# Hongje/OTVM

Hardware: AMD Instinct MI355X
Metric: frames_per_sec (higher is better)
Workload: dtype f16x3 (fp32 operands split into fp16 hi+lo, fp32 accumulate); 1 GPU; synthetic 1920x1080 clip, T=140 frames (untimed lead-in 0 + warmup 5 + timed: the last 135), memory every 5, max 5 slots, trimap propagation + alpha + memorize per frame, one sequence per GPU; weights=synthetic (otvm_amd.synth_weights seed 0), parallelism=sequence-per-gpu x1, batch=1

## Files before the change

### include/otvm_hip.h

```cpp
#ifndef OTVM_HIP_H
#define OTVM_HIP_H

#include <stdint.h>

#ifdef __cplusplus
extern "C" {
#endif

#define OTVM_ACT_NONE 0
#define OTVM_ACT_RELU 1
#define OTVM_ACT_LEAKY 2

#define OTVM_PREC_F32 0
#define OTVM_PREC_F16X3 1
#define OTVM_PREC_F16 2

const char* otvm_last_error(void);
#define OTVM_ABI_VERSION 21
int otvm_abi_version(void);

int otvm_pack_conv_weight(const float* w_oihw, int O, int I, int kh, int kw, int ws, const float* scale,
                          float* w_packed, int O_pad, int I_pad, int K_pad, void* stream);

int64_t otvm_patch_weight_bytes_f16x3(int O, int I_pad);
// ... 58 lines not shown
int otvm_conv2d_candidates(const otvm_conv_params* p, int* out, int max_n);
int otvm_conv2d_accepts_input_norm(const otvm_conv_params* p);
int otvm_conv2d_input_norm_kind(const otvm_conv_params* p);

typedef struct otvm_conv_up_params {
    const float* src; int Hi, Wi, Cu, src_ld;
    int64_t src_bs;
    const float* scale; const float* shift;
    int act;
    int norm_bs;
    int tile_rows;
} otvm_conv_up_params;
int otvm_conv2d_up(const otvm_conv_params* p, const otvm_conv_up_params* u, void* stream);
int otvm_conv2d_accepts_upsampled_input(const otvm_conv_params* p, const otvm_conv_up_params* u);

int otvm_split_conv_weight_f16x3(const float* w_packed, int O, int O_pad, int K_pad, int taps, int I_pad,
                                 void* w_hi, void* w_lo, float* w_scale, void* stream);

int64_t otvm_wave_weight_bytes_f16x3(int O_pad, int K_pad);
int otvm_pack_wave_weight_f16x3(const void* w_hi, const void* w_lo, int O_pad, int K_pad, void* w_wfrag, void* stream);

typedef struct {
    const float* x; int H, W, Cin, x_ld;
    float* y; int y_ld;
    const void* w1f; const void* w2f; const void* w3f;
    const float* s1; const float* s2; const float* s3;
    const float* b1; const float* b2; const float* b3;
    int batch; int64_t x_bs, y_bs;
    int tile;
} otvm_stm_bottleneck_params;
// ... 4 lines not shown
                  float* shift, void* stream);
int otvm_gn_apply(const float* x, int64_t P, int C, int ld, const double* stats, const float* gamma,
                  const float* beta, const float* residual, int res_ld, const float* res_scale, const float* res_shift,
                  int res_act, int act, float* out, int out_ld, void* stream);

int otvm_gn_stats_b(const float* x, int64_t P, int C, int ld, double* stats, int batch, int64_t x_bs, int stats_bs, void* stream);
int otvm_gn_table_b(const double* stats, int64_t P, int C, const float* gamma, const float* beta, float* scale, float* shift,
                    int batch, int stats_bs, int norm_bs, void* stream);
typedef struct {
    const float* x; int64_t P; int C, ld; const double* stats; const float* gamma; const float* beta;
    const float* residual; int res_ld; const float* res_scale; const float* res_shift; int res_act, act;
    float* out; int out_ld;
    int batch; int64_t x_bs, res_bs, out_bs; int stats_bs, norm_bs;
} otvm_gn_apply_params;
int otvm_gn_apply_b(const otvm_gn_apply_params* p, void* stream);

typedef struct otvm_gram_params {
    const float* x; int64_t P; int C, ld;
    const float* in_scale; const float* in_shift; int in_act;
    float* gpart; float* spart; int passes;
    int batch; int64_t x_bs; int norm_bs;
    unsigned* diag;
} otvm_gram_params;
int otvm_gram_block(int C);
int64_t otvm_gram_entries(int C);
int otvm_gram_chunks(int64_t P, int C, int* pch_out);
int otvm_gram_f16(const otvm_gram_params* p, void* stream);
typedef struct otvm_gn_predict_params {
    const float* gpart; const float* spart; int64_t P; int C, Cout;
    const float* Mp; const double* v; void* ws; unsigned* counter;
// ... 270 lines not shown
```

### otvm_amd/csrc/conv_stem_f16x3.hip

```cpp
#include "common.h"
#include "f16x3_ops.h"
#include <type_traits>
#include <stdlib.h>

namespace {

struct StemArgs {
    const float* in; const _Float16* wf; const float* wscale; const float* bias; float* out; double* gn_stats;
    int H, W, Cin, in_ld, Ho, Wo, Cout, out_ld, act, groups;
    int tiles_x, tiles_y; OtvmTileWalk walk;
    int64_t in_bs, out_bs; int gn_bs;
    OtvmGnTail tail;
};

constexpr int TH = 8, TW = 32, NW = 4, NT = NW * 64;
constexpr int TM = TH / NW, TN = 2;
constexpr int PH = 2 * TH + 5, PW = 2 * TW + 5, NPIX = PH * PW;
constexpr int KSTEPS = 25;

__global__ __launch_bounds__(NT) __attribute__((amdgpu_waves_per_eu(2, 2))) void conv_stem_f16x3_kernel(const StemArgs pa) {
    StemArgs p = pa;
    {
        const int zb = blockIdx.y;
        p.in += zb * p.in_bs;
        p.out += zb * p.out_bs;
        if (p.gn_stats) p.gn_stats += zb * p.gn_bs;
    }
    constexpr int PATCH_HALFS = 2 * NPIX * 8;
    constexpr int EPI_HALFS = NW * 32 * 36 * 2;
    constexpr int SM_HALFS = PATCH_HALFS > EPI_HALFS ? PATCH_HALFS : EPI_HALFS;
    __shared__ __attribute__((aligned(16))) _Float16 smem[SM_HALFS];
    _Float16* Ph = smem;
    _Float16* Pl = smem + NPIX * 8;

    const int tid = threadIdx.x, lane = tid & 63, wave = tid >> 6;
    int tile_n_, tile_x, tile_y;
    otvm_tile_decode(p.walk, blockIdx.x, gridDim.x, 1, p.tiles_x, p.tiles_y, tile_n_, tile_x, tile_y);
    const int ty0 = tile_y * TH, tx0 = tile_x * TW;
    const int iy00 = 2 * ty0 - 3, ix00 = 2 * tx0 - 3;

    f32x16 acc[TM][TN];
// ... 151 lines not shown
                        const int64_t m = (int64_t)y * p.Wo + x;
                        if (FULL || (vec_ok && n4 + 3 < p.Cout)) {
                            v.x = otvm_act(v.x, p.act); v.y = otvm_act(v.y, p.act);
                            v.z = otvm_act(v.z, p.act); v.w = otvm_act(v.w, p.act);
                            *reinterpret_cast<f32x4*>(p.out + m * p.out_ld + n4) = v;
                        } else {
#pragma unroll
                            for (int j = 0; j < 4; ++j)
                                if (n4 + j < p.Cout) p.out[m * p.out_ld + n4 + j] = otvm_act(v[j], p.act);
                        }
                    }
                }
            }
        }
    };
    if (interior) {
        if (p.act == OTVM_ACT_RELU) epilogue_full(std::integral_constant<int, OTVM_ACT_RELU>{});
        else if (p.act == OTVM_ACT_LEAKY) epilogue_full(std::integral_constant<int, OTVM_ACT_LEAKY>{});
        else epilogue_full(std::integral_constant<int, OTVM_ACT_NONE>{});
    } else {
        epilogue(std::false_type{});
    }
    if (p.gn_stats) {
        __shared__ double gred[2 * 64];
        const int cg = p.Cout >> 5;
        const int seg = cg < 32 ? cg : 32;
        for (int i = tid; i < 2 * 64; i += NT) gred[i] = 0.0;
        __syncthreads();
#pragma unroll
        for (int b = 0; b < TN; ++b) {
            const int n = b * 32 + col;
            float s = 0.f, ss = 0.f, cnt = 0.f;
            const float pil = n < p.Cout && p.bias ? p.bias[n / cg * cg] : 0.f;
            if (n < p.Cout) {
                const float sc_ = p.wscale[n];
                const float bias = p.bias ? p.bias[n] : 0.f, bd = bias - pil;
// ... 25 lines not shown
                double S, SS;
                otvm_gn_unshift(s, ss, (int)cnt, pil, S, SS);
                atomicAdd(&gred[2 * gl], S);
                atomicAdd(&gred[2 * gl + 1], SS);
            }
        }
        __syncthreads();
        const int ng = (64 + cg - 1) / cg;
        for (int i = tid; i < 2 * ng; i += NT) {
            const int g = i >> 1;
            if (g < 32 && gred[i] != 0.0) atomicAdd(&p.gn_stats[2 * g + (i & 1)], gred[i]);
        }
        __syncthreads();
        otvm_gn_table_tail(p.gn_stats, (int64_t)p.Ho * p.Wo, p.Cout, p.tail, blockIdx.y, gridDim.x, reinterpret_cast<float*>(gred));
    }
}

__global__ __launch_bounds__(256) void pack_stem_weight_kernel(const float* __restrict__ w, int O, int K_pad, int I_pad, int groups,
                                                               _Float16* __restrict__ wf, float* __restrict__ wscale) {
    const int n = blockIdx.x;
    __shared__ float red[256];
    const bool real = n < O;
    const float* row = w + (int64_t)n * K_pad;
    float mx = 0.f;
    if (real)
        for (int k = threadIdx.x; k < 49 * I_pad; k += 256) mx = fmaxf(mx, fabsf(row[k]));
    red[threadIdx.x] = mx;
    __syncthreads();
    for (int s = 128; s > 0; s >>= 1) {
        if (threadIdx.x < s) red[threadIdx.x] = fmaxf(red[threadIdx.x], red[threadIdx.x + s]);
// ... 38 lines not shown
                   p->Cin <= 64 && !p->residual && !p->in_relu && !p->in_scale ? 1 : 0;
}

int otvm_conv2d_stem_f16x3(const otvm_conv_params* p, void* stream) {
    StemArgs a;
    a.in = p->in; a.wf = (const _Float16*)p->w_frag; a.wscale = p->w_scale; a.bias = p->bias; a.out = p->out;
    a.gn_stats = p->gn_stats;
    a.tail = otvm_gn_tail_of(p);
    a.H = p->H; a.W = p->W; a.Cin = p->Cin; a.in_ld = p->in_ld; a.Ho = p->Ho; a.Wo = p->Wo; a.Cout = p->Cout;
    a.out_ld = p->out_ld; a.act = p->act; a.groups = (p->Cin + 7) / 8;
    a.tiles_x = otvm_ceil_div(p->Wo, TW);
    a.tiles_y = otvm_ceil_div(p->Ho, TH);
    a.walk = otvm_tile_walk_of(2);
    const int batch = p->batch > 1 ? p->batch : 1;
    a.in_bs = batch > 1 ? p->in_bs : 0; a.out_bs = batch > 1 ? p->out_bs : 0; a.gn_bs = batch > 1 ? p->gn_bs : 0;
    hipLaunchKernelGGL(conv_stem_f16x3_kernel, dim3(a.tiles_x * a.tiles_y, batch), dim3(NT), 0, (hipStream_t)stream, a);
    OTVM_CHECK_LAUNCH("otvm_conv2d(stem f16x3)");
    return 0;
}
```

### otvm_amd/csrc/groupnorm.hip

```cpp
#include "common.h"
#include "f16x3_ops.h"
#include <stdlib.h>

namespace {

constexpr int G = 32;

__global__ void gn_stats_kernel(const float* __restrict__ x, int64_t P, int C, int ld, double* __restrict__ stats,
                                int64_t x_bs, int stats_bs) {
    x += blockIdx.y * x_bs;
    stats += blockIdx.y * stats_bs;
    __shared__ double red[G * 2];
    const int Q = C >> 2;
    const int rows = blockDim.x / Q;
    const int q = threadIdx.x % Q, r = threadIdx.x / Q;
    if (threadIdx.x < G * 2) red[threadIdx.x] = 0.0;
    __syncthreads();
    f32x4 s = {0.f, 0.f, 0.f, 0.f}, ss = {0.f, 0.f, 0.f, 0.f}, p0 = {0.f, 0.f, 0.f, 0.f};
    int n = 0;
    const int64_t pix0 = (int64_t)blockIdx.x * rows + r, step = (int64_t)gridDim.x * rows;
    if (r < rows && pix0 < P) {
        p0 = *reinterpret_cast<const f32x4*>(x + pix0 * ld + q * 4);
        n = (int)((P - 1 - pix0) / step) + 1;
        int64_t pix = pix0 + step;
// ... 81 lines not shown
        rb = *reinterpret_cast<const f32x4*>(res_shift + c);
    }
    for (; pix < P; pix += dpix) {
        f32x4 v = *reinterpret_cast<const f32x4*>(x + pix * ld + c);
        v = v * a + b;
        if (residual) {
            f32x4 r = *reinterpret_cast<const f32x4*>(residual + pix * res_ld + c);
            if (res_scale) {
                r = r * ra + rb;
                r.x = otvm_act(r.x, res_act); r.y = otvm_act(r.y, res_act); r.z = otvm_act(r.z, res_act); r.w = otvm_act(r.w, res_act);
            }
            v += r;
        }
        v.x = otvm_act(v.x, act); v.y = otvm_act(v.y, act); v.z = otvm_act(v.z, act); v.w = otvm_act(v.w, act);
        *reinterpret_cast<f32x4*>(out + pix * out_ld + c) = v;
    }
}

__global__ void gn_table_kernel(const double* __restrict__ stats, int64_t P, int C, const float* __restrict__ gamma,
                                const float* __restrict__ beta, float* __restrict__ scale, float* __restrict__ shift,
                                int stats_bs, int norm_bs) {
    stats += blockIdx.x * stats_bs;
    scale += blockIdx.x * norm_bs;
    shift += blockIdx.x * norm_bs;
    __shared__ float mean_s[G], rstd_s[G];
    const int cg = C / G;
    if (threadIdx.x < G) {
        const double cnt = (double)P * cg;
        const double mean = stats[threadIdx.x * 2] / cnt;
        double var = stats[threadIdx.x * 2 + 1] / cnt - mean * mean;
// ... 61 lines not shown
    const int64_t total = q->P * Q;
    int64_t blocks = (total + 255) / 256;
    if (blocks > 4096) blocks = 4096;
    int gcd = 256, r = Q;
    while (r) { const int t = gcd % r; gcd = r; r = t; }
    const int m = Q / gcd;
    blocks = (blocks + m - 1) / m * m;
    const bool b = batch > 1;
    hipLaunchKernelGGL(gn_apply_kernel, dim3((int)blocks, batch), dim3(256), 0, (hipStream_t)stream, q->x, q->P, C, q->ld, q->stats,
                       q->gamma, q->beta, q->residual, q->res_ld, q->res_scale, q->res_shift, q->res_act, q->act, q->out, q->out_ld,
                       b ? q->x_bs : 0, b ? q->res_bs : 0, b ? q->out_bs : 0, b ? q->stats_bs : 0, b ? q->norm_bs : 0);
    OTVM_CHECK_LAUNCH("otvm_gn_apply");
    return 0;
}

extern "C" int otvm_gn_apply(const float* x, int64_t P, int C, int ld, const double* stats, const float* gamma,
                             const float* beta, const float* residual, int res_ld, const float* res_scale,
                             const float* res_shift, int res_act, int act, float* out, int out_ld, void* stream) {
    otvm_gn_apply_params q;
    q.x = x; q.P = P; q.C = C; q.ld = ld; q.stats = stats; q.gamma = gamma; q.beta = beta; q.residual = residual; q.res_ld = res_ld;
    q.res_scale = res_scale; q.res_shift = res_shift; q.res_act = res_act; q.act = act; q.out = out; q.out_ld = out_ld;
    q.batch = 1; q.x_bs = q.res_bs = q.out_bs = 0; q.stats_bs = q.norm_bs = 0;
    return otvm_gn_apply_b(&q, stream);
}
```

### otvm_amd/engine.py

```python
import ctypes as C
import os

import torch

from . import lib as L

NONE, RELU, LEAKY = 0, 1, 2
GUARD_CLEAR = 2 ** 31 - 1
F16_LIMIT = 65504.0
FUSE_GN_STATS = True
FUSE_GN_APPLY = os.environ.get("OTVM_FUSE_GN_APPLY", "1") != "0"
_GRAPHS_ENV = os.environ.get("OTVM_GRAPHS")
USE_GRAPHS = None if _GRAPHS_ENV in (None, "", "auto") else (_GRAPHS_ENV != "0")
GRAPH_AUTO_PIXELS = 1 << 22


def graphs_wanted(setting, padded_pixels):
    if setting is not None:
        return bool(setting)
    if int(os.environ.get("WORLD_SIZE", "1")) > 1:
        return True
    return padded_pixels < GRAPH_AUTO_PIXELS
PRE_ON_S2 = os.environ.get("OTVM_PRE_ON_S2", "1") != "0"
EVDEC_LATE = os.environ.get("OTVM_EVDEC_LATE", "1") != "0"
WAVE_TILE = os.environ.get("OTVM_WAVE_TILE", "0") != "0"
FUSE_GN_APPLY_IGEMM = os.environ.get("OTVM_FUSE_GN_APPLY_IGEMM", "1") != "0"
FUSE_GN_APPLY_IGEMM_KXK = os.environ.get("OTVM_FUSE_GN_APPLY_IGEMM_KXK", "0") != "0"
FUSE_GN_TABLE = os.environ.get("OTVM_FUSE_GN_TABLE", "1") != "0"
FUSE_STM_BLOCK = os.environ.get("OTVM_FUSE_STM_BLOCK", "1") != "0"
FUSE_STM_BLOCK128 = int(os.environ.get("OTVM_FUSE_STM_BLOCK128", "1"))
STM128_TILE = int(os.environ.get("OTVM_STM128_TILE", "0"))
FOLD_UPSAMPLE = int(os.environ.get("OTVM_FOLD_UPSAMPLE", "1"))
FUSE_PPM_HEAD = os.environ.get("OTVM_PPM_HEAD", "1") != "0"
FUSE_GN_PREDICT = os.environ.get("OTVM_GN_PREDICT", "1") != "0"
GN_PREDICT_MIN_PIXELS = int(os.environ.get("OTVM_GN_PREDICT_MIN_PIXELS", "16384"))
GN_PREDICT_PASSES = int(os.environ.get("OTVM_GN_PREDICT_PASSES", "1"))
GN_PREDICT_PLANES = tuple(int(v) for v in os.environ.get("OTVM_GN_PREDICT_PLANES", "64,128,256,512").split(",") if v)
GN_PREDICT_DS = os.environ.get("OTVM_GN_PREDICT_DS", "1") != "0"
GN_PREDICT_KAPPA_P3 = float(os.environ.get("OTVM_GN_PREDICT_KAPPA_P3", "4"))
GN_PREDICT_KAPPA_OFF = float(os.environ.get("OTVM_GN_PREDICT_KAPPA_OFF", "256"))
FUSE_REFINE_TAIL = os.environ.get("OTVM_FUSE_REFINE_TAIL", "0") != "0"
FUSE_HEAD = os.environ.get("OTVM_FUSE_HEAD", "1") != "0"
HEAD16 = os.environ.get("OTVM_HEAD16", "1") != "0"
PPM_ALGEBRA = os.environ.get("OTVM_PPM_ALGEBRA", "1") != "0"


AUTOTUNE = os.environ.get("OTVM_AUTOTUNE", "1") != "0"
# ... 948 lines not shown
        self.H, self.W, self.B = H, W, B
        self.fgr = bool(eng._fgr_on)
        if B > 1 and eng.precision != L.PREC_F16X3:
            raise NotImplementedError("otvm_amd: batched sequences (B > 1) run on the f16x3 path only")
        self.lw, self.uw, self.lh, self.uh = pad_amounts(H, W, 32)
        self.Hp, self.Wp = H + self.lh + self.uh, W + self.lw + self.uw
        self.P = self.Hp * self.Wp
        self._bufs = {}
        self._keep = []
        self.graphs, self._graph_warm = {}, {}
        self._n_conv = {}
        self._retired_graphs = []
        self._stm128 = []
        self._upfold = []
        self.upfold_routes = {}
        self._fused_stats = []
        self._convs = []
        self._predicted = []
        self.diag = None
        self.n_gn = 0
        self.steps = {}
        self._build()
        self.stats_bs = max(self.n_gn, 1) * 64
        self.stats = torch.zeros(self.B * self.stats_bs, dtype=torch.float64, device=self.dev)
        self._bind_stats()
        self.autotune()

    @staticmethod
    def _signature(p):
        return (p.H, p.W, p.Cin, p.in_ld, p.Cout, p.out_ld, p.kh, p.kw, p.stride, p.pad, p.dil, p.in_relu, p.act, int(bool(p.bias)),
# ... 44 lines not shown
                                 forced=(STM128_TILE or -1) if FUSE_STM_BLOCK128 >= 2 else None, default=None if timed else -1)
                if choice == 0:
                    S[i:i + 1] = U
                    i += len(U)
                else:
                    q.tile = max(choice, 0)
                    S[i] = fused
                    i += 1
        self._stm128 = []
        _save_choices_timed_since(n_logged)

    def autotune(self):
        if not (AUTOTUNE and self.e.precision == L.PREC_F16X3):
            self._resolve_stm128(timed=False)
            self._resolve_upfold(timed=False)
            return
        filled = []
        gen = torch.Generator(device=self.dev)
        gen.manual_seed(0x07F3)
        for b in self._bufs.values():
            t = b.t if isinstance(b, Act) else b
            if not t.is_floating_point():
                continue
            if t.dtype == torch.float32:
                t.normal_(generator=gen)
            else:
                continue
            filled.append(t)
        H16, W16 = self.Hp // 16, self.Wp // 16
        tk = Act(torch.empty(self.B * self.hw * 128, dtype=torch.float32, device=self.dev), H16, W16, 128, B=self.B, bs=self.hw * 128)
        tv = Act(torch.empty(self.B * self.hw * 512, dtype=torch.float32, device=self.dev), H16, W16, 512, B=self.B, bs=self.hw * 512)
        n0, k0 = len(self._convs), len(self._keep)
        self.conv([], self.r4m, "trimap.model.KV_M_r4.Key", tk, pad=1)
        self.conv([], self.r4m, "trimap.model.KV_M_r4.Value", tv, pad=1)
        self.tune_convs(self._convs)
        self._resolve_stm128(timed=FUSE_STM_BLOCK128 == 1)
        torch.cuda.synchronize(self.dev)
        del self._convs[n0:], self._keep[k0:]
        self._resolve_upfold(timed=FOLD_UPSAMPLE == 1)
        torch.cuda.synchronize(self.dev)
        for t in filled:
            t.zero_()
        self.stats.zero_()
        torch.cuda.synchronize(self.dev)

    def retire_graphs(self):
        self._retired_graphs.extend(self.graphs.values())
        self.graphs, self._graph_warm = {}, {}

    def clear_stats(self, stream):
        L.check(self.lib.otvm_clear(self.stats.data_ptr(), self.stats.numel() * 8, stream), "clear GroupNorm statistics")

    def buf(self, name, H, W, C):
        key = (name, H, W, C)
# ... 122 lines not shown
        for key, S in self.steps.items():
            for i, st in enumerate(S):
                if st[0] == "gn_stats":
                    _, a, idx, (nb, x_bs), label = st
                    S[i] = (self.lib.otvm_gn_stats_b, a + (base + idx * 512, nb, x_bs, sbs), label)
                elif st[0] == "gn_table":
                    _, a, idx, nbs, label = st
                    S[i] = (self.lib.otvm_gn_table_b, (base + idx * 512,) + a + (self.B, sbs, nbs), label)
                elif st[0] == "ppm_add":
                    _, a, b, label = st
                    S[i] = (self.lib.otvm_ppm_conv_add, a + (self._ppm_stats.gn_stats + 8 * b * sbs,), label)
                elif st[0] == "gn_apply":
                    _, q, idx, label = st
                    q.stats, q.stats_bs = base + idx * 512, sbs
                    S[i] = (self.lib.otvm_gn_apply_b, (C.byref(q),), label)

    def upsample(self, S, x, out, add=None, norm=None):
        S.append((self.lib.otvm_upsample_bilinear_b,
                  (x.ptr, x.H, x.W, x.C, x.ld, 0 if norm is None else norm[0], 0 if norm is None else norm[1],
                   0 if norm is None else norm[2], 0 if add is None else add.ptr, 0 if add is None else add.ld,
                   out.ptr, out.H, out.W, out.ld, x.B, x.bs, 0 if add is None else add.bs, out.bs,
                   0 if norm is None else norm[3]), "upsample"))

    def gn_then_upsample(self, S, x, gn_name, gn_act, producer_p, out):
        if FUSE_GN_APPLY and FUSE_GN_STATS and producer_p is not None:
            sc, sh, nbs = self.gn_table_step(S, x, gn_name, producer_p)
            self.upsample(S, x, out, norm=(sc, sh, gn_act, nbs))
            m = {"name": gn_name, "S": S, "step": S[-1], "src": x, "norm": (sc, sh, gn_act, nbs), "out": out, "readers": []}
            self._upfold.append(m)
            return m
# ... 31 lines not shown
                             lambda: _time_candidates(self.e, _EventClock(self.dev), routes.get, (0, 1) * 4, 3, warm=(0, 0, 1, 1)),
                             forced=1 if FOLD_UPSAMPLE >= 2 else None, default=None if timed else 0)
            if choice:
                at = lambda S, st: next(i for i, q in enumerate(S) if q is st)
                del m["S"][at(m["S"], m["step"])]
                for (S, step, p, x, wname), fs in zip(m["readers"], folded):
                    S[at(S, step)] = fs
                self.upfold_routes[m["name"]] = 1
                for b in range(max(1, m["out"].B)):
                    m["out"].torch(b).zero_()
        self._upfold = []
        _save_choices_timed_since(n_logged)

    def maxpool(self, S, x, out):
        S.append((self.lib.otvm_maxpool3x3s2_b, (x.ptr, x.H, x.W, x.C, x.ld, out.ptr, out.ld, x.B, x.bs, out.bs), "maxpool"))

    def gn_bottleneck(self, S, x, p, planes, stride, dil, has_ds, out):
        Ho, Wo = x.H // stride, x.W // stride
        t1 = self.buf("bt1", x.H, x.W, planes)
        cp = self.conv(S, x, p + ".conv1", t1)
        t2 = self.buf("bt2", Ho, Wo, planes)
        cp = self.gn_then_conv(S, t1, p + ".bn1", RELU, cp, p + ".conv2", t2, stride=stride, pad=dil, dil=dil)
        if self._predicted_tail(S, x, p, planes, stride, has_ds, out, t2, cp):
            return
        t3 = self.buf("bt3", Ho, Wo, planes * 4)
        if FUSE_GN_APPLY_IGEMM:
            cp3 = self.gn_then_conv(S, t2, p + ".bn2", RELU, cp, p + ".conv3", t3)
        else:
            self.gn(S, t2, p + ".bn2", RELU, conv_p=cp)
            cp3 = self.conv(S, t2, p + ".conv3", t3)
# ... 105 lines not shown
        self.conv(U, t2, p + ".conv3", out, residual=idt, act=RELU)
        if fuse128:
            q = L.StmBottleneckParams(x.ptr, x.H, x.W, x.C, x.ld, out.ptr, out.ld,
                                      c1.w_wfrag.data_ptr(), c2.w_wfrag.data_ptr(), c3.w_wfrag.data_ptr(),
                                      c1.w_scale.data_ptr(), c2.w_scale.data_ptr(), c3.w_scale.data_ptr(),
                                      c1.bias.data_ptr(), c2.bias.data_ptr(), c3.bias.data_ptr(), x.B, x.bs, out.bs, 0)
            self._keep.append(q)
            P = x.B * x.H * x.W
            flops = 2 * P * (512 * 128 + 9 * 128 * 128 + 128 * 512)
            abytes = 4 * (P * 512 * 2 + 512 * 128 * 2 + 9 * 128 * 128)
            fused = (self.lib.otvm_stm_bottleneck_f16x3, (C.byref(q),), "conv " + p + " (fused bottleneck)", flops, abytes,
                     (x, out.ch(0, 512) if out.C > 512 else out))
            S.append(("stm128", fused, U, q, p))
            self._stm128.append(S)

    def stm_trunk(self, S, stem_out, e, tag):
        H4, W4 = self.Hp // 4, self.Wp // 4
        x = self.buf(tag + "pool", H4, W4, 64)
        self.maxpool(S, stem_out, x)
        outs = {}
        for lname, n, planes, s0 in (("res2", 3, 64, 1), ("res3", 4, 128, 2), ("res4", 6, 256, 2)):
            for b in range(n):
                st = s0 if b == 0 else 1
                o = self.buf(tag + lname + ("a" if b % 2 == 0 else "b"), x.H // st, x.W // st, planes * 4)
                self.bn_bottleneck(S, x, e + "%s.%d" % (lname, b), planes, st, b == 0, o, tag)
                x = o
            outs[lname] = x
        return outs["res4"], outs["res3"], outs["res2"]

    def resblock(self, S, x, p, out, tag):
        r = self.buf(tag + "r", x.H, x.W, 256)
        self.conv(S, x, p + ".conv1", r, pad=1, in_relu=1)
        self.conv(S, r, p + ".conv2", out, pad=1, in_relu=1, residual=x)

# ... 9 lines not shown
        self.SQ = self.buf("SQ", Hp, Wp, 4)
        self.SMs = [self.buf("SM0", Hp, Wp, 24), self.buf("SM1", Hp, Wp, 24)]
        self.D80 = self.buf("D80", Hp, Wp, 80)
        self.PROBS_B = self.raws("probs", 3 * P)
        self.CLS_B = self.raws("cls", P, torch.uint8)
        self.ALPHA_P_B = self.raws("alpha_p", P)
        self.TRI_P_B = self.raws("tri_p", 3 * P)
        self.FGR_P_B = self.raws("fgr_p", 3 * P) if self.fgr else None
        self.enc_ws_B = self.raws("enc_ws", _rup(int(lib.otvm_trimap_encode_ws_bytes(Hp, Wp)), 256), torch.uint8)
        self.PROBS, self.CLS, self.ALPHA_P, self.TRI_P = self.PROBS_B[0], self.CLS_B[0], self.ALPHA_P_B[0], self.TRI_P_B[0]

        S = []
        sd = e.sd
        q = "trimap.model.Encoder_Q."
        stem = self.buf("q_stem", H2, W2, 64)
        self.conv(S, self.SQ, q + "conv1", stem, stride=2, pad=3, act=RELU)
        r4, r3, r2 = self.stm_trunk(S, stem, q, "q_")
        self.QK = self.buf("QK", H16, W16, 128)
        self.M4 = self.buf("M4", H16, W16, 1024)
        self.conv(S, r4, "trimap.model.KV_Q_r4.Key", self.QK, pad=1)
        self.conv(S, r4, "trimap.model.KV_Q_r4.Value", self.M4.ch(512, 512), pad=1)
        self.steps["segment_a"] = S
        self._ws = self.SPLITK_WS[0]
        S = []
        d = "trimap.model.Decoder."
        SK = []
        self._ws = self.SPLITK_WS[3]
        skips = {}
        for rf, feat, (h, w) in (("RF3", r3, (H8, W8)), ("RF2", r2, (H4, W4))):
            s0 = self.buf("d_s0", h, w, 256)
            self.conv(SK, feat, d + rf + ".convFS", s0, pad=1)
            s1 = self.buf("d_s1", h, w, 256)
# ... 15 lines not shown
        self.L4 = self.buf("L4", H4, W4, 4)
        self.conv(S, pm, d + "pred", self.L4, pad=1, in_relu=1)
        for b in range(self.B):
            S.append((lib.otvm_upsample4_softmax3, (self.L4.img(b).ptr, H4, W4, self.L4.ld, self.PROBS_B[b].data_ptr()), "up4softmax"))
        self.steps["segment_b"] = S

        S = []
        en = "NET.encoder."
        self.U3 = self.buf("U3", H2, W2, 320)
        self.U2 = self.buf("U2", H4, W4, 512)
        ppm_alg = FUSE_PPM_HEAD and self.e.W_ppm is not None
        self.PPMCAT = self.buf("PPMCAT", H8, W8, 2048 if ppm_alg else 3072)
        c1raw = self.buf("c1raw", H2, W2, 64)
        cp = self.conv(S, self.X11, en + "conv1", c1raw, stride=2, pad=3)
        c1 = self.U3.ch(256, 64)
        self.gn(S, c1raw, en + "bn1", RELU, out=c1, conv_p=cp)
        x = self.buf("e_pool", H4, W4, 64)
        self.maxpool(S, c1, x)
        cfg = {"layer1": (64, 3, 1, 1, 1), "layer2": (128, 4, 2, 1, 1), "layer3": (256, 6, 1, 1, 2),
               "layer4": (512, 3, 1, 2, 4)}
        for lname in ("layer1", "layer2", "layer3", "layer4"):
            planes, n, s0, d0, dn = cfg[lname]
            for b in range(n):
                st = s0 if b == 0 else 1
                last = b == n - 1
                if last and lname == "layer1":
                    o = self.U2.ch(256, 256)
                elif last and lname == "layer4":
                    o = self.PPMCAT.ch(0, 2048)
                else:
                    o = self.buf("e_" + lname + ("a" if b % 2 == 0 else "b"), x.H // st, x.W // st, planes * 4)
                self.gn_bottleneck(S, x, en + "%s.%d" % (lname, b), planes, st, d0 if b == 0 else dn, b == 0, o)
                x = o
# ... 117 lines not shown
                continue
            self.conv(S, h32, rf + "pred.2", hid, pad=1, act=LEAKY)
            for b in range(self.B):
                args = (hid.img(b).ptr, hid.ld, sd[rf + "pred.4.weight"].data_ptr(), sd[rf + "pred.4.bias"].data_ptr(), 10,
                        img.img(b).ptr, img.ld, P, self.ALPHA_P_B[b].data_ptr(), 1, self.TRI_P_B[b].data_ptr(),
                        SM.ch(16, 8).img(b).ptr, SM.ld)
                if self.fgr:
                    S.append((lib.otvm_fba_head_fgr, args + (self.FGR_P_B[b].data_ptr(),), "fba_head10 (+ F)"))
                else:
                    S.append((lib.otvm_fba_head, args, "fba_head10"))
            self.steps["fba_tail%d" % par] = S

        self._ws = self.SPLITK_WS[1]
        m_ = "trimap.model.Encoder_M."
        stem = self.buf("m_stem", H2, W2, 64)
        for par in (0, 1):
            S = []
            self.conv(S, self.SMs[par], m_ + "stem", stem, stride=2, pad=3, act=RELU)
            self.steps["mem_stem%d" % par] = S
        S = []
        self.r4m, _, _ = self.stm_trunk(S, stem, m_, "m_")
        self.steps["mem_trunk"] = S
        self.mem_ws = None

    def run(self, key, stream, tstream=None):
        prof = self.e.prof
        nc = self._n_conv.get(key)
        if nc is None:
            nc = self._n_conv[key] = sum(1 for st in self.steps[key] if not isinstance(st[0], str) and st[2].startswith("conv "))
        self.e.conv_calls += nc
        if prof is None and self.e.check_level >= 3:
            for st in self.steps[key]:
                if isinstance(st[0], str):
                    continue
                if st[2].startswith("conv "):
                    self.e.guard(st[5][0], "input of " + st[2], stream)
# ... 160 lines not shown
```

### otvm_amd/lib.py

```python
import ctypes as C
import os

_HERE = os.path.dirname(os.path.abspath(__file__))
LIB_PATH = os.environ.get("OTVM_HIP_LIB") or os.path.join(_HERE, "libotvm_hip.so")

vp, i32, i64, f32 = C.c_void_p, C.c_int, C.c_int64, C.c_float
PREC_F32, PREC_F16X3, PREC_F16 = 0, 1, 2
ABI_VERSION = 21


class ConvParams(C.Structure):
    _fields_ = [("inp", vp), ("H", i32), ("W", i32), ("Cin", i32), ("in_ld", i32),
                ("w", vp), ("K_pad", i32),
                ("bias", vp),
                ("residual", vp), ("res_ld", i32),
                ("out", vp), ("Ho", i32), ("Wo", i32), ("Cout", i32), ("out_ld", i32),
                ("kh", i32), ("kw", i32), ("stride", i32), ("pad", i32), ("dil", i32),
                ("in_relu", i32), ("act", i32),
                ("precision", i32), ("w_hi", vp), ("w_lo", vp), ("w_scale", vp), ("w_frag", vp),
                ("gn_stats", vp),
                ("in_scale", vp), ("in_shift", vp), ("in_act", i32),
                ("tune", i32),
                ("splitk_ws", vp), ("splitk_ws_bytes", i64),
                ("batch", i32), ("in_bs", i64), ("out_bs", i64), ("res_bs", i64), ("gn_bs", i32), ("norm_bs", i32),
# ... 7 lines not shown
    _fields_ = [("src", vp), ("Hi", i32), ("Wi", i32), ("Cu", i32), ("src_ld", i32), ("src_bs", i64),
                ("scale", vp), ("shift", vp), ("act", i32), ("norm_bs", i32), ("tile_rows", i32)]


class StmBottleneckParams(C.Structure):
    _fields_ = [("x", vp), ("H", i32), ("W", i32), ("Cin", i32), ("x_ld", i32), ("y", vp), ("y_ld", i32),
                ("w1f", vp), ("w2f", vp), ("w3f", vp), ("s1", vp), ("s2", vp), ("s3", vp), ("b1", vp), ("b2", vp), ("b3", vp),
                ("batch", i32), ("x_bs", i64), ("y_bs", i64), ("tile", i32)]


class GnApplyParams(C.Structure):
    _fields_ = [("x", vp), ("P", i64), ("C", i32), ("ld", i32), ("stats", vp), ("gamma", vp), ("beta", vp),
                ("residual", vp), ("res_ld", i32), ("res_scale", vp), ("res_shift", vp), ("res_act", i32), ("act", i32),
                ("out", vp), ("out_ld", i32),
                ("batch", i32), ("x_bs", i64), ("res_bs", i64), ("out_bs", i64), ("stats_bs", i32), ("norm_bs", i32)]


class HeadParams(C.Structure):
    _fields_ = [("w", vp), ("b", vp), ("n_out", i32), ("img", vp), ("img_ld", i32), ("P", i64), ("alpha_out", vp),
                ("alpha_stride", i32), ("tri_out", vp), ("sm", vp), ("sm_ld", i32),
                ("img_bs", i64), ("alpha_bs", i64), ("tri_bs", i64), ("sm_bs", i64), ("w16", vp)]


class GramParams(C.Structure):
    _fields_ = [("x", vp), ("P", i64), ("C", i32), ("ld", i32), ("in_scale", vp), ("in_shift", vp), ("in_act", i32),
                ("gpart", vp), ("spart", vp), ("passes", i32), ("batch", i32), ("x_bs", i64), ("norm_bs", i32), ("diag", vp)]


class GnPredictParams(C.Structure):
    _fields_ = [("gpart", vp), ("spart", vp), ("P", i64), ("C", i32), ("Cout", i32), ("Mp", vp), ("v", vp), ("ws", vp),
# ... 178 lines not shown
    "otvm_loss_fba_comp": (i32, [vp, vp, vp, vp, vp, vp, i64, i64, vp, vp, vp, vp, vp, vp]),
    "otvm_loss_grad_l1": (i32, [vp, vp, i64, i32, i32, f32, vp, vp]),
    "otvm_loss_exclusion_level": (i32, [vp, vp, i32, i32, i32, i32, f32, vp, vp, vp]),
    "otvm_avgpool2": (i32, [vp, i64, i32, i32, vp, vp]),
    "otvm_loss_lap_level": (i32, [vp, vp, i64, i32, i32, C.c_double, vp, vp, vp, vp]),
    "otvm_loss_temporal": (i32, [vp, vp, i32, i32, i64, vp, vp]),
    "otvm_loss_ce3": (i32, [vp, vp, i64, i64, vp, vp]),
    "otvm_finite_guard": (i32, [vp, i64, i32, i32, f32, i32, vp, vp]),
    "otvm_clear": (i32, [vp, i64, vp]),
    "otvm_gram_block": (i32, [i32]),
    "otvm_gram_entries": (i64, [i32]),
    "otvm_gram_chunks": (i32, [i64, i32, C.POINTER(i32)]),
    "otvm_gram_f16": (i32, [C.POINTER(GramParams), vp]),
    "otvm_gn_predict": (i32, [C.POINTER(GnPredictParams), vp]),
    "otvm_gn_predict_ws_bytes": (i64, []),
}

EXPORTED = sorted(list(_PROTOS) + ["otvm_last_error"])

_lib = None


def load():
    global _lib
    if _lib is not None:
        return _lib
    if not os.path.exists(LIB_PATH):
        raise RuntimeError(
            "otvm_amd: %s is missing -- build it with `python otvm_amd/csrc/build.py` "
            "(or __graft_entry__.build()).  There is no CPU/PyTorch fallback." % LIB_PATH)
# ... 20 lines not shown
```

Measured before the change: 46.79 frames/s.

## Fold 3x3 stride-2 max-pool into stem conv epilogue and GroupNorm apply

```diff
diff --git a/include/otvm_hip.h b/include/otvm_hip.h
--- a/include/otvm_hip.h
+++ b/include/otvm_hip.h
@@ -96,6 +96,9 @@
 int otvm_conv2d_up(const otvm_conv_params* p, const otvm_conv_up_params* u, void* stream);
 int otvm_conv2d_accepts_upsampled_input(const otvm_conv_params* p, const otvm_conv_up_params* u);
 
+int otvm_conv2d_accepts_stem_pool(const otvm_conv_params* p);
+int otvm_conv2d_stem_pool(const otvm_conv_params* p, float* pool, int pool_ld, int64_t pool_bs, void* stream);
+
 int otvm_split_conv_weight_f16x3(const float* w_packed, int O, int O_pad, int K_pad, int taps, int I_pad,
                                  void* w_hi, void* w_lo, float* w_scale, void* stream);
 
@@ -130,6 +133,12 @@
     int batch; int64_t x_bs, res_bs, out_bs; int stats_bs, norm_bs;
 } otvm_gn_apply_params;
 int otvm_gn_apply_b(const otvm_gn_apply_params* p, void* stream);
+typedef struct {
+    const float* x; int H, W, C, ld; const double* stats; const float* gamma; const float* beta; int act;
+    float* out; int out_ld; float* pool; int pool_ld;
+    int batch; int64_t x_bs, out_bs, pool_bs; int stats_bs;
+} otvm_gn_apply_maxpool_params;
+int otvm_gn_apply_maxpool_b(const otvm_gn_apply_maxpool_params* p, void* stream);
 
 typedef struct otvm_gram_params {
     const float* x; int64_t P; int C, ld;
diff --git a/otvm_amd/csrc/conv_stem_f16x3.hip b/otvm_amd/csrc/conv_stem_f16x3.hip
--- a/otvm_amd/csrc/conv_stem_f16x3.hip
+++ b/otvm_amd/csrc/conv_stem_f16x3.hip
@@ -11,6 +11,7 @@
     int tiles_x, tiles_y; OtvmTileWalk walk;
     int64_t in_bs, out_bs; int gn_bs;
     OtvmGnTail tail;
+    float* pool; int pool_ld, Hq, Wq; int64_t pool_bs;
 };
 
 constexpr int TH = 8, TW = 32, NW = 4, NT = NW * 64;
@@ -18,13 +19,15 @@
 constexpr int PH = 2 * TH + 5, PW = 2 * TW + 5, NPIX = PH * PW;
 constexpr int KSTEPS = 25;
 
+template <bool POOL>
 __global__ __launch_bounds__(NT) __attribute__((amdgpu_waves_per_eu(2, 2))) void conv_stem_f16x3_kernel(const StemArgs pa) {
     StemArgs p = pa;
     {
         const int zb = blockIdx.y;
         p.in += zb * p.in_bs;
-        p.out += zb * p.out_bs;
+        if (!POOL || p.out) p.out += zb * p.out_bs;
         if (p.gn_stats) p.gn_stats += zb * p.gn_bs;
+        if (POOL) p.pool += zb * p.pool_bs;
     }
     constexpr int PATCH_HALFS = 2 * NPIX * 8;
     constexpr int EPI_HALFS = NW * 32 * 36 * 2;
@@ -206,12 +209,64 @@
             }
         }
     };
-    if (interior) {
-        if (p.act == OTVM_ACT_RELU) epilogue_full(std::integral_constant<int, OTVM_ACT_RELU>{});
-        else if (p.act == OTVM_ACT_LEAKY) epilogue_full(std::integral_constant<int, OTVM_ACT_LEAKY>{});
-        else epilogue_full(std::integral_constant<int, OTVM_ACT_NONE>{});
-    } else {
-        epilogue(std::false_type{});
+    if (!POOL || p.out) {
+        if (interior) {
+            if (p.act == OTVM_ACT_RELU) epilogue_full(std::integral_constant<int, OTVM_ACT_RELU>{});
+            else if (p.act == OTVM_ACT_LEAKY) epilogue_full(std::integral_constant<int, OTVM_ACT_LEAKY>{});
+            else epilogue_full(std::integral_constant<int, OTVM_ACT_NONE>{});
+        } else {
+            epilogue(std::false_type{});
+        }
+    }
+    if constexpr (POOL) {
+        if (p.out) __syncthreads();
+        float* T = reinterpret_cast<float*>(smem);
+        static_assert(TH * TW * 36 * 4 <= SM_HALFS * 2, "the pooled epilogue's tile does not fit the patch buffer");
+        const int py0 = ty0 >> 1, px0 = tx0 >> 1;
+#pragma unroll
+        for (int b = 0; b < TN; ++b) {
+            const float sc = p.wscale[b * 32 + col], bi = p.bias ? p.bias[b * 32 + col] : 0.f;
+#pragma unroll
+            for (int a = 0; a < TM; ++a) {
+                const int row = wave * TM + a;
+#pragma unroll
+                for (int e = 0; e < 16; ++e) {
+                    const int xi = (e & 3) + 8 * (e >> 2) + rbase;
+                    float v = otvm_act(acc[a][b][e] * sc + bi, OTVM_ACT_RELU);
+                    if (ty0 + row >= p.Ho || tx0 + xi >= p.Wo) v = 0.f;
+                    T[(row * TW + xi) * 36 + col] = v;
+                }
+            }
+            __syncthreads();
+            for (int i = tid; i < 5 * 17 * 8; i += NT) {
+                const int q4 = (i & 7) * 4, pp = i >> 3, pk = pp / 17, pj = pp - pk * 17;
+                const int gy = py0 + pk, gx = px0 + pj;
+                if (gy >= p.Hq || gx >= p.Wq) continue;
+                f32x4 m = {0.f, 0.f, 0.f, 0.f};
+#pragma unroll
+                for (int dy = -1; dy <= 1; ++dy) {
+                    const int r = min(max(2 * pk + dy, 0), TH - 1);
+#pragma unroll
+                    for (int dx = -1; dx <= 1; ++dx) {
+                        const int cc = min(max(2 * pj + dx, 0), TW - 1);
+                        const f32x4 t = *reinterpret_cast<const f32x4*>(&T[(r * TW + cc) * 36 + q4]);
+                        m.x = fmaxf(m.x, t.x); m.y = fmaxf(m.y, t.y); m.z = fmaxf(m.z, t.z); m.w = fmaxf(m.w, t.w);
+                    }
+                }
+                float* dst = p.pool + ((int64_t)gy * p.Wq + gx) * p.pool_ld + b * 32 + q4;
+                if (pk >= 1 && pk <= 3 && pj >= 1 && pj <= 15) {
+                    *reinterpret_cast<f32x4*>(dst) = m;
+                } else {
+#pragma unroll
+                    for (int j = 0; j < 4; ++j)
+                        if (m[j] > 0.f)
+                            __hip_atomic_fetch_max(reinterpret_cast<unsigned*>(dst + j), __float_as_uint(m[j]), __ATOMIC_RELAXED,
+                                                   __HIP_MEMORY_SCOPE_AGENT);
+                }
+            }
+            __syncthreads();
+        }
+        return;
     }
     if (p.gn_stats) {
         __shared__ double gred[2 * 64];
@@ -267,6 +322,16 @@
         __syncthreads();
         otvm_gn_table_tail(p.gn_stats, (int64_t)p.Ho * p.Wo, p.Cout, p.tail, blockIdx.y, gridDim.x, reinterpret_cast<float*>(gred));
     }
+}
+
+__global__ __launch_bounds__(256) void stem_pool_clear_kernel(float* __restrict__ pool, int Hq, int Wq, int pool_ld, int64_t pool_bs) {
+    pool += blockIdx.y * pool_bs;
+    const int64_t i = (int64_t)blockIdx.x * 256 + threadIdx.x;
+    const int64_t pix = i >> 4;
+    if (pix >= (int64_t)Hq * Wq) return;
+    const int gy = (int)(pix / Wq), gx = (int)(pix - (int64_t)gy * Wq);
+    if ((gy % (TH / 2)) != 0 && (gx % (TW / 2)) != 0) return;
+    *reinterpret_cast<f32x4*>(pool + pix * pool_ld + (int)(i & 15) * 4) = f32x4{0.f, 0.f, 0.f, 0.f};
 }
 
 __global__ __launch_bounds__(256) void pack_stem_weight_kernel(const float* __restrict__ w, int O, int K_pad, int I_pad, int groups,
@@ -335,7 +400,48 @@
     a.walk = otvm_tile_walk_of(2);
     const int batch = p->batch > 1 ? p->batch : 1;
     a.in_bs = batch > 1 ? p->in_bs : 0; a.out_bs = batch > 1 ? p->out_bs : 0; a.gn_bs = batch > 1 ? p->gn_bs : 0;
-    hipLaunchKernelGGL(conv_stem_f16x3_kernel, dim3(a.tiles_x * a.tiles_y, batch), dim3(NT), 0, (hipStream_t)stream, a);
+    a.pool = nullptr; a.pool_ld = a.Hq = a.Wq = 0; a.pool_bs = 0;
+    hipLaunchKernelGGL(conv_stem_f16x3_kernel<false>, dim3(a.tiles_x * a.tiles_y, batch), dim3(NT), 0, (hipStream_t)stream, a);
     OTVM_CHECK_LAUNCH("otvm_conv2d(stem f16x3)");
     return 0;
 }
+
+extern "C" int otvm_conv2d_accepts_stem_pool(const otvm_conv_params* p) {
+    if (!p || !otvm_prec_is_split(p->precision) || !p->in || !p->w_scale || !otvm_conv2d_stem_eligible(p)) return 0;
+    if (p->act != OTVM_ACT_RELU || p->gn_stats || p->gn_scale_out || p->in_res || p->Cout != 64) return 0;
+    if (p->tune && p->tune / 16 - 1 != 12) return 0;
+    if (p->Cin % 4 != 0 || p->in_ld % 4 != 0 || ((uintptr_t)p->in & 15) || p->in_ld < p->Cin) return 0;
+    if (p->H < 1 || p->W < 1 || p->Ho != (p->H - 1) / 2 + 1 || p->Wo != (p->W - 1) / 2 + 1) return 0;
+    if (p->out && (p->out_ld < 64)) return 0;
+    if (p->batch > 1 && ((p->in_bs & 3) || (p->out && (p->out_bs & 3)))) return 0;
+    return 1;
+}
+
+extern "C" int otvm_conv2d_stem_pool(const otvm_conv_params* p, float* pool, int pool_ld, int64_t pool_bs, void* stream) {
+    OTVM_REQUIRE(p && pool, "otvm_conv2d_stem_pool: null pointer");
+    OTVM_REQUIRE(otvm_conv2d_accepts_stem_pool(p),
+                 "otvm_conv2d_stem_pool: needs an f16x3 7x7 stride-2 stem with 64 filters, ReLU and no GroupNorm statistics "
+                 "(otvm_conv2d_accepts_stem_pool)");
+    const int batch = p->batch > 1 ? p->batch : 1;
+    OTVM_REQUIRE(pool_ld >= 64 && pool_ld % 4 == 0 && ((uintptr_t)pool & 15) == 0 && (batch == 1 || (pool_bs > 0 && pool_bs % 4 == 0)),
+                 "otvm_conv2d_stem_pool: the pooled view needs 16-byte aligned pixels of >= 64 floats");
+    StemArgs a;
+    a.in = p->in; a.wf = (const _Float16*)p->w_frag; a.wscale = p->w_scale; a.bias = p->bias; a.out = p->out;
+    a.gn_stats = nullptr;
+    a.tail = otvm_gn_tail_of(p);
+    a.H = p->H; a.W = p->W; a.Cin = p->Cin; a.in_ld = p->in_ld; a.Ho = p->Ho; a.Wo = p->Wo; a.Cout = p->Cout;
+    a.out_ld = p->out_ld; a.act = p->act; a.groups = (p->Cin + 7) / 8;
+    a.tiles_x = otvm_ceil_div(p->Wo, TW);
+    a.tiles_y = otvm_ceil_div(p->Ho, TH);
+    a.walk = otvm_tile_walk_of(2);
+    a.in_bs = batch > 1 ? p->in_bs : 0; a.out_bs = batch > 1 ? p->out_bs : 0; a.gn_bs = 0;
+    a.pool = pool; a.pool_ld = pool_ld; a.Hq = (p->Ho - 1) / 2 + 1; a.Wq = (p->Wo - 1) / 2 + 1;
+    a.pool_bs = batch > 1 ? pool_bs : 0;
+    const int64_t nclear = (int64_t)a.Hq * a.Wq * 16;
+    hipLaunchKernelGGL(stem_pool_clear_kernel, dim3((unsigned)((nclear + 255) / 256), batch), dim3(256), 0, (hipStream_t)stream, pool, a.Hq,
+                       a.Wq, pool_ld, a.pool_bs);
+    OTVM_CHECK_LAUNCH("otvm_conv2d_stem_pool (clear)");
+    hipLaunchKernelGGL(conv_stem_f16x3_kernel<true>, dim3(a.tiles_x * a.tiles_y, batch), dim3(NT), 0, (hipStream_t)stream, a);
+    OTVM_CHECK_LAUNCH("otvm_conv2d_stem_pool");
+    return 0;
+}
diff --git a/otvm_amd/csrc/groupnorm.hip b/otvm_amd/csrc/groupnorm.hip
--- a/otvm_amd/csrc/groupnorm.hip
+++ b/otvm_amd/csrc/groupnorm.hip
@@ -119,6 +119,76 @@
         }
         v.x = otvm_act(v.x, act); v.y = otvm_act(v.y, act); v.z = otvm_act(v.z, act); v.w = otvm_act(v.w, act);
         *reinterpret_cast<f32x4*>(out + pix * out_ld + c) = v;
+    }
+}
+
+__global__ __launch_bounds__(256) void gn_apply_maxpool_kernel(const float* __restrict__ x, int H, int W, int C, int ld,
+                                                               const double* __restrict__ stats, const float* __restrict__ gamma,
+                                                               const float* __restrict__ beta, int act, float* __restrict__ out,
+                                                               int out_ld, float* __restrict__ pool, int Ho, int Wo, int pool_ld,
+                                                               int64_t x_bs, int64_t out_bs, int64_t pool_bs, int stats_bs) {
+    {
+        const int zb = blockIdx.y;
+        x += zb * x_bs;
+        out += zb * out_bs;
+        pool += zb * pool_bs;
+        stats += zb * stats_bs;
+    }
+    __shared__ float mean_s[G], rstd_s[G];
+    const int cg = C / G;
+    if (threadIdx.x < G) {
+        const double cnt = (double)((int64_t)H * W) * cg;
+        const double mean = stats[threadIdx.x * 2] / cnt;
+        double var = stats[threadIdx.x * 2 + 1] / cnt - mean * mean;
+        if (var < 0.0) var = 0.0;
+        mean_s[threadIdx.x] = (float)mean;
+        rstd_s[threadIdx.x] = (float)(1.0 / sqrt(var + 1e-5));
+    }
+    __syncthreads();
+    const int Q = C >> 2;
+    const int64_t i0 = (int64_t)blockIdx.x * blockDim.x + threadIdx.x;
+    const int64_t NP = (int64_t)Ho * Wo;
+    int64_t pix = i0 / Q;
+    const int c = (int)(i0 - pix * Q) * 4;
+    const int64_t dpix = (int64_t)gridDim.x * blockDim.x / Q;
+    f32x4 a, b;
+#pragma unroll
+    for (int j = 0; j < 4; ++j) {
+        const int g = (c + j) / cg;
+        a[j] = rstd_s[g] * gamma[c + j];
+        b[j] = beta[c + j] - mean_s[g] * a[j];
+    }
+    const float ninf = -__builtin_huge_valf();
+    for (; pix < NP; pix += dpix) {
+        const int oy = (int)(pix / Wo), ox = (int)(pix - (int64_t)oy * Wo);
+        f32x4 v[3][3];
+#pragma unroll
+        for (int dy = 0; dy < 3; ++dy) {
+            const int iy = oy * 2 + dy - 1;
+#pragma unroll
+            for (int dx = 0; dx < 3; ++dx) {
+                const int ix = ox * 2 + dx - 1;
+                v[dy][dx] = f32x4{0.f, 0.f, 0.f, 0.f};
+                if ((unsigned)iy < (unsigned)H && (unsigned)ix < (unsigned)W)
+                    v[dy][dx] = *reinterpret_cast<const f32x4*>(x + ((int64_t)iy * W + ix) * ld + c);
+            }
+        }
+        f32x4 m = {ninf, ninf, ninf, ninf};
+#pragma unroll
+        for (int dy = 0; dy < 3; ++dy) {
+            const int iy = oy * 2 + dy - 1;
+#pragma unroll
+            for (int dx = 0; dx < 3; ++dx) {
+                const int ix = ox * 2 + dx - 1;
+                if ((unsigned)iy >= (unsigned)H || (unsigned)ix >= (unsigned)W) continue;
+                f32x4 t = v[dy][dx];
+                t = t * a + b;
+                t.x = otvm_act(t.x, act); t.y = otvm_act(t.y, act); t.z = otvm_act(t.z, act); t.w = otvm_act(t.w, act);
+                m.x = fmaxf(m.x, t.x); m.y = fmaxf(m.y, t.y); m.z = fmaxf(m.z, t.z); m.w = fmaxf(m.w, t.w);
+                if (dy >= 1 && dx >= 1) *reinterpret_cast<f32x4*>(out + ((int64_t)iy * W + ix) * out_ld + c) = t;
+            }
+        }
+        *reinterpret_cast<f32x4*>(pool + pix * pool_ld + c) = m;
     }
 }
 
@@ -210,6 +280,28 @@
     return 0;
 }
 
+extern "C" int otvm_gn_apply_maxpool_b(const otvm_gn_apply_maxpool_params* q, void* stream) {
+    OTVM_REQUIRE(q && q->x && q->out && q->pool && q->stats && q->gamma && q->beta, "otvm_gn_apply_maxpool: null pointer");
+    const int C = q->C;
+    OTVM_REQUIRE(C % 64 == 0 && 1024 % C == 0, "otvm_gn_apply_maxpool: C=%d unsupported (64, 128, 256, 512 or 1024)", C);
+    OTVM_REQUIRE(q->H >= 1 && q->W >= 1, "otvm_gn_apply_maxpool: empty map");
+    OTVM_REQUIRE(q->ld % 4 == 0 && q->out_ld % 4 == 0 && q->pool_ld % 4 == 0 && q->ld >= C && q->out_ld >= C && q->pool_ld >= C &&
+                 ((uintptr_t)q->x & 15) == 0 && ((uintptr_t)q->out & 15) == 0 && ((uintptr_t)q->pool & 15) == 0,
+                 "otvm_gn_apply_maxpool: unaligned view");
+    const int batch = q->batch > 1 ? q->batch : 1;
+    OTVM_REQUIRE(batch == 1 || (q->x_bs % 4 == 0 && q->out_bs % 4 == 0 && q->pool_bs % 4 == 0),
+                 "otvm_gn_apply_maxpool: batch strides must be multiples of 4 elements");
+    const int Ho = (q->H - 1) / 2 + 1, Wo = (q->W - 1) / 2 + 1;
+    int64_t blocks = ((int64_t)Ho * Wo * (C / 4) + 255) / 256;
+    if (blocks > 4096) blocks = 4096;
+    const bool b = batch > 1;
+    hipLaunchKernelGGL(gn_apply_maxpool_kernel, dim3((int)blocks, batch), dim3(256), 0, (hipStream_t)stream, q->x, q->H, q->W, C,
+                       q->ld, q->stats, q->gamma, q->beta, q->act, q->out, q->out_ld, q->pool, Ho, Wo, q->pool_ld, b ? q->x_bs : 0,
+                       b ? q->out_bs : 0, b ? q->pool_bs : 0, b ? q->stats_bs : 0);
+    OTVM_CHECK_LAUNCH("otvm_gn_apply_maxpool");
+    return 0;
+}
+
 extern "C" int otvm_gn_apply(const float* x, int64_t P, int C, int ld, const double* stats, const float* gamma,
                              const float* beta, const float* residual, int res_ld, const float* res_scale,
                              const float* res_shift, int res_act, int act, float* out, int out_ld, void* stream) {
diff --git a/otvm_amd/engine.py b/otvm_amd/engine.py
--- a/otvm_amd/engine.py
+++ b/otvm_amd/engine.py
@@ -31,6 +31,8 @@
 FUSE_STM_BLOCK128 = int(os.environ.get("OTVM_FUSE_STM_BLOCK128", "1"))
 STM128_TILE = int(os.environ.get("OTVM_STM128_TILE", "0"))
 FOLD_UPSAMPLE = int(os.environ.get("OTVM_FOLD_UPSAMPLE", "1"))
+FOLD_POOL = os.environ.get("OTVM_FOLD_POOL", "1") != "0"
+FOLD_STEM_POOL = int(os.environ.get("OTVM_FOLD_STEM_POOL", "1"))
 FUSE_PPM_HEAD = os.environ.get("OTVM_PPM_HEAD", "1") != "0"
 FUSE_GN_PREDICT = os.environ.get("OTVM_GN_PREDICT", "1") != "0"
 GN_PREDICT_MIN_PIXELS = int(os.environ.get("OTVM_GN_PREDICT_MIN_PIXELS", "16384"))
@@ -1009,6 +1011,9 @@
         self._stm128 = []
         self._upfold = []
         self.upfold_routes = {}
+        self._stempool = []
+        self.stempool_routes = {}
+        self.poolfold_routes = {}
         self._fused_stats = []
         self._convs = []
         self._predicted = []
@@ -1083,6 +1088,7 @@
         if not (AUTOTUNE and self.e.precision == L.PREC_F16X3):
             self._resolve_stm128(timed=False)
             self._resolve_upfold(timed=False)
+            self._resolve_stempool(timed=False)
             return
         filled = []
         gen = torch.Generator(device=self.dev)
@@ -1107,6 +1113,7 @@
         torch.cuda.synchronize(self.dev)
         del self._convs[n0:], self._keep[k0:]
         self._resolve_upfold(timed=FOLD_UPSAMPLE == 1)
+        self._resolve_stempool(timed=FOLD_STEM_POOL == 1)
         torch.cuda.synchronize(self.dev)
         for t in filled:
             t.zero_()
@@ -1259,6 +1266,10 @@
                     _, q, idx, label = st
                     q.stats, q.stats_bs = base + idx * 512, sbs
                     S[i] = (self.lib.otvm_gn_apply_b, (C.byref(q),), label)
+                elif st[0] == "gn_apply_pool":
+                    _, q, idx, label = st
+                    q.stats, q.stats_bs = base + idx * 512, sbs
+                    S[i] = (self.lib.otvm_gn_apply_maxpool_b, (C.byref(q),), label)
 
     def upsample(self, S, x, out, add=None, norm=None):
         S.append((self.lib.otvm_upsample_bilinear_b,
@@ -1320,6 +1331,64 @@
 
     def maxpool(self, S, x, out):
         S.append((self.lib.otvm_maxpool3x3s2_b, (x.ptr, x.H, x.W, x.C, x.ld, out.ptr, out.ld, x.B, x.bs, out.bs), "maxpool"))
+
+    def gn_then_maxpool(self, S, x, name, act, out, pooled, conv_p=None):
+        self.poolfold_routes[name] = int(FOLD_POOL)
+        if not FOLD_POOL:
+            self.gn(S, x, name, act, out=out, conv_p=conv_p)
+            self.maxpool(S, out, pooled)
+            return
+        sd = self.e.sd
+        idx = self.n_gn
+        self.n_gn += 1
+        if conv_p is not None and FUSE_GN_STATS:
+            self._fused_stats.append((conv_p, idx))
+        else:
+            S.append(("gn_stats", (x.ptr, x.P, x.C, x.ld), idx, (self.B, x.bs), "gn_stats " + name))
+        q = L.GnApplyMaxpoolParams()
+        q.x, q.H, q.W, q.C, q.ld = x.ptr, x.H, x.W, x.C, x.ld
+        q.gamma, q.beta, q.act = sd[name + ".weight"].data_ptr(), sd[name + ".bias"].data_ptr(), act
+        q.out, q.out_ld, q.pool, q.pool_ld = out.ptr, out.ld, pooled.ptr, pooled.ld
+        q.batch, q.x_bs, q.out_bs, q.pool_bs = self.B, x.bs, out.bs, pooled.bs
+        self._keep.append(q)
+        S.append(("gn_apply_pool", q, idx, "gn_apply " + name + " (+ maxpool)"))
+
+    def _resolve_stempool(self, timed):
+        n_logged = len(TUNE_LOG)
+        for m in self._stempool:
+            self.stempool_routes[m["name"]] = 0
+            if FOLD_STEM_POOL <= 0:
+                continue
+            pooled, folded = m["pooled"], []
+            for S, step, p, x in m["stems"]:
+                pf = L.ConvParams()
+                C.memmove(C.byref(pf), C.byref(p), C.sizeof(L.ConvParams))
+                pf.out, pf.out_ld, pf.out_bs = 0, 0, 0
+                if not self.lib.otvm_conv2d_accepts_stem_pool(C.byref(pf)):
+                    folded = None
+                    break
+                self._keep.append(pf)
+                saved = 4 * x.B * (p.Ho * p.Wo - pooled.H * pooled.W) * p.Cout
+                folded.append((self.lib.otvm_conv2d_stem_pool, (C.byref(pf), pooled.ptr, pooled.ld, pooled.bs), step[2] + " (+ maxpool)",
+                               step[3], step[4] - saved, (x, pooled)))
+            if folded is None:
+                continue
+            (_, step0, p0, x0), (SP, pool_step) = m["stems"][0], m["pool"]
+            key = (-4, p0.H, p0.W, max(1, x0.B), p0.Cin, p0.in_ld, p0.Cout, pooled.ld)
+            routes = {0: [step0, pool_step], 1: [folded[0]]}
+            choice = _choose(key, m["name"] + " (stem + max-pool: 0 = two launches, 1 = pooled map written by the stem)",
+                             (p0.H, p0.W, p0.Cin, p0.in_ld, p0.Cout, pooled.ld, 7, 7, 2, 3, 1),
+                             lambda: _time_candidates(self.e, _EventClock(self.dev), routes.get, (0, 1) * 4, 3, warm=(0, 0, 1, 1)),
+                             forced=1 if FOLD_STEM_POOL >= 2 else None, default=None if timed else 0,
+                             settle=lambda ms, fastest: fastest if ms[fastest] <= 0.97 * ms[0] else 0)
+            if choice:
+                at = lambda S, st: next(i for i, q in enumerate(S) if q is st)
+                del SP[at(SP, pool_step)]
+                for (S, step, p, x), fs in zip(m["stems"], folded):
+                    S[at(S, step)] = fs
+                self.stempool_routes[m["name"]] = 1
+        self._stempool = []
+        _save_choices_timed_since(n_logged)
 
     def gn_bottleneck(self, S, x, p, planes, stride, dil, has_ds, out):
         Ho, Wo = x.H // stride, x.W // stride
@@ -1455,10 +1524,12 @@
             S.append(("stm128", fused, U, q, p))
             self._stm128.append(S)
 
-    def stm_trunk(self, S, stem_out, e, tag):
+    def stm_trunk(self, S, stem_out, e, tag, stems=None):
         H4, W4 = self.Hp // 4, self.Wp // 4
         x = self.buf(tag + "pool", H4, W4, 64)
         self.maxpool(S, stem_out, x)
+        if stems is not None:
+            self._stempool.append({"name": stems[0], "stems": stems[1], "pool": (S, S[-1]), "pooled": x})
         outs = {}
         for lname, n, planes, s0 in (("res2", 3, 64, 1), ("res3", 4, 128, 2), ("res4", 6, 256, 2)):
             for b in range(n):
@@ -1498,8 +1569,8 @@
         sd = e.sd
         q = "trimap.model.Encoder_Q."
         stem = self.buf("q_stem", H2, W2, 64)
-        self.conv(S, self.SQ, q + "conv1", stem, stride=2, pad=3, act=RELU)
-        r4, r3, r2 = self.stm_trunk(S, stem, q, "q_")
+        cp = self.conv(S, self.SQ, q + "conv1", stem, stride=2, pad=3, act=RELU)
+        r4, r3, r2 = self.stm_trunk(S, stem, q, "q_", stems=(q + "conv1", [(S, S[-1], cp, self.SQ)]))
         self.QK = self.buf("QK", H16, W16, 128)
         self.M4 = self.buf("M4", H16, W16, 1024)
         self.conv(S, r4, "trimap.model.KV_Q_r4.Key", self.QK, pad=1)
@@ -1545,9 +1616,8 @@
         c1raw = self.buf("c1raw", H2, W2, 64)
         cp = self.conv(S, self.X11, en + "conv1", c1raw, stride=2, pad=3)
         c1 = self.U3.ch(256, 64)
-        self.gn(S, c1raw, en + "bn1", RELU, out=c1, conv_p=cp)
         x = self.buf("e_pool", H4, W4, 64)
-        self.maxpool(S, c1, x)
+        self.gn_then_maxpool(S, c1raw, en + "bn1", RELU, c1, x, conv_p=cp)
         cfg = {"layer1": (64, 3, 1, 1, 1), "layer2": (128, 4, 2, 1, 1), "layer3": (256, 6, 1, 1, 2),
                "layer4": (512, 3, 1, 2, 4)}
         for lname in ("layer1", "layer2", "layer3", "layer4"):
@@ -1695,12 +1765,14 @@
         self._ws = self.SPLITK_WS[1]
         m_ = "trimap.model.Encoder_M."
         stem = self.buf("m_stem", H2, W2, 64)
+        stems = []
         for par in (0, 1):
             S = []
-            self.conv(S, self.SMs[par], m_ + "stem", stem, stride=2, pad=3, act=RELU)
+            cp = self.conv(S, self.SMs[par], m_ + "stem", stem, stride=2, pad=3, act=RELU)
+            stems.append((S, S[-1], cp, self.SMs[par]))
             self.steps["mem_stem%d" % par] = S
         S = []
-        self.r4m, _, _ = self.stm_trunk(S, stem, m_, "m_")
+        self.r4m, _, _ = self.stm_trunk(S, stem, m_, "m_", stems=(m_ + "stem", stems))
         self.steps["mem_trunk"] = S
         self.mem_ws = None
 
diff --git a/otvm_amd/lib.py b/otvm_amd/lib.py
--- a/otvm_amd/lib.py
+++ b/otvm_amd/lib.py
@@ -45,6 +45,12 @@
                 ("residual", vp), ("res_ld", i32), ("res_scale", vp), ("res_shift", vp), ("res_act", i32), ("act", i32),
                 ("out", vp), ("out_ld", i32),
                 ("batch", i32), ("x_bs", i64), ("res_bs", i64), ("out_bs", i64), ("stats_bs", i32), ("norm_bs", i32)]
+
+
+class GnApplyMaxpoolParams(C.Structure):
+    _fields_ = [("x", vp), ("H", i32), ("W", i32), ("C", i32), ("ld", i32), ("stats", vp), ("gamma", vp), ("beta", vp), ("act", i32),
+                ("out", vp), ("out_ld", i32), ("pool", vp), ("pool_ld", i32),
+                ("batch", i32), ("x_bs", i64), ("out_bs", i64), ("pool_bs", i64), ("stats_bs", i32)]
 
 
 class HeadParams(C.Structure):
@@ -253,6 +259,9 @@
     "otvm_gram_f16": (i32, [C.POINTER(GramParams), vp]),
     "otvm_gn_predict": (i32, [C.POINTER(GnPredictParams), vp]),
     "otvm_gn_predict_ws_bytes": (i64, []),
+    "otvm_gn_apply_maxpool_b": (i32, [C.POINTER(GnApplyMaxpoolParams), vp]),
+    "otvm_conv2d_accepts_stem_pool": (i32, [C.POINTER(ConvParams)]),
+    "otvm_conv2d_stem_pool": (i32, [C.POINTER(ConvParams), vp, i32, i64, vp]),
 }
 
 EXPORTED = sorted(list(_PROTOS) + ["otvm_last_error"])
```

New measurement: 46.85 frames/s, median of 5. No clear change (+0.1%).
